# volivan239/raytracing-course-hw

Measured on AMD Instinct MI355X. Metric: Msamples/sec at 1920x1080x256spp, higher is better.
Workload: dtype f32; 1 GPU; synth_room_v1_1920x1080x256; scene=synth_room_v1 (seed 20241223), triangles=268816, emissive_triangles=4204, width=1920, height=1080, spp=256, ray_depth=6, parallelism=pixel tiles 32x32 round-robin over 1 GPU(s), bvh_nodes=265605, bvh_depth=24, light_bvh_depth=19, device_bytes=120573816

## Files before the change

### raytracing-course-hw_amd/csrc/device/rt_persistent.h

```cpp
#pragma once
#include "rt_wavefront.h"

namespace rtamd {
namespace dev {

#define P8_WAVES 4
#define P8_THREADS (64 * P8_WAVES)
#define P8_PER_CU 5
#define PT_MAX_PATHS 5120
#define PT_MIN_GROUP 16
#define PT_NW (PT_MAX_PATHS / 32)
#define PT_BIT_T 1u
#define PT_BIT_L 2u
#define PT_NONE 0xFFFFFFFFu
#define PT_Q_TRACE 0
#define PT_Q_LIGHT 1
#define PT_Q_SHADE 2
#define PT_Q_XLIGHT 3
#define PT_Q_XTRACE 4
#define PT_N_LIVE 5
#define PT_W_TRACE 6
#define PT_W_LIGHT 7
#define PT_GSHIFT 15
#define PT_COST_TRACE_NODE 1u
#define PT_COST_TRACE_TRI 1u
#define PT_COST_LIGHT_NODE 2u
#define PT_COST_LIGHT_TEST 2u
#define PT_COST_SHADE 14u
#define PT_DEBUG_BLOCKS 2048
#define PT_DRAINED 0xFFFFFFFEu
#define PT_T_OVERFLOW (-1.f)
#define PT_WIDE_NONE 0
#define PT_WIDE_WENT 1
#define PT_WIDE_FULL 2
RT_DEV uint32_t pt_near_key(bool entered, uint32_t key) { return entered ? key : 0xFFFFFFFFu; }
RT_DEV void pt_order(uint32_t &ka, uint32_t &ca, uint32_t &kb, uint32_t &cb) {
    const bool s = kb < ka;
    const uint32_t k = s ? kb : ka, c = s ? cb : ca;
    kb = s ? ka : kb; cb = s ? ca : cb;
    ka = k; ca = c;
}
RT_DEV int pt_wide_step_nearest(const GpuNode4Q *nodes, const RayGrid &ray, float cull_t, uint32_t (*stack)[64], int lane, int &sp, int cap, uint32_t &cur) {
    const uint4 *q = reinterpret_cast<const uint4 *>(nodes + cur);
    const uint4 b0 = q[0], b1 = q[1], b2 = q[2], b3 = q[3];
    uint32_t k0, k1, k2, k3;
    const bool h0 = slab_enter_q(b0, ray, cull_t, k0), h1 = slab_enter_q(b1, ray, cull_t, k1);
    const bool h2 = slab_enter_q(b2, ray, cull_t, k2), h3 = slab_enter_q(b3, ray, cull_t, k3);
    k0 = pt_near_key(h0, k0); k1 = pt_near_key(h1, k1); k2 = pt_near_key(h2, k2); k3 = pt_near_key(h3, k3);
    uint32_t c0 = b0.w, c1 = b1.w, c2 = b2.w, c3 = b3.w;
    pt_order(k0, c0, k1, c1); pt_order(k2, c2, k3, c3); pt_order(k0, c0, k2, c2); pt_order(k1, c1, k3, c3); pt_order(k1, c1, k2, c2);
    const int nh = (int)h0 + (int)h1 + (int)h2 + (int)h3;
    if (nh == 0) return PT_WIDE_NONE;
    if (sp + nh - 1 > cap) return PT_WIDE_FULL;
    if (nh > 3) stack[sp++][lane] = c3;
    if (nh > 2) stack[sp++][lane] = c2;
    if (nh > 1) stack[sp++][lane] = c1;
    cur = c0;
    return PT_WIDE_WENT;
}
RT_DEV void pt_wide_enter_all(const GpuNode4Q *nodes, uint32_t cur, const RayGrid &ray, uint4 &b0, uint4 &b1, uint4 &b2, uint4 &b3,
                              bool &h0, bool &h1, bool &h2, bool &h3) {
    const uint4 *q = reinterpret_cast<const uint4 *>(nodes + cur);
    b0 = q[0]; b1 = q[1]; b2 = q[2]; b3 = q[3];
    h0 = slab_test_q(b0, ray); h1 = slab_test_q(b1, ray); h2 = slab_test_q(b2, ray); h3 = slab_test_q(b3, ray);
}
RT_DEV int pt_wide_step_all(const GpuNode4Q *nodes, const RayGrid &ray, uint32_t (*stack)[64], int lane, int &sp, int cap, uint32_t &cur) {
    uint4 b0, b1, b2, b3;
// ... 16 lines not shown
    bool h[4];
    pt_wide_enter_all(S.light_walk_nodes4, 0u, ray, b[0], b[1], b[2], b[3], h[0], h[1], h[2], h[3]);
    steps = 1;
    if (!(h[0] | h[1] | h[2] | h[3])) return 0;
    if (LEVELS < 2) return 2;
    for (int c = 0; c < 4; c++) {
        if (!h[c]) continue;
        if (b[c].w & RT_LEAF_BIT) return 2;
        uint4 g0, g1, g2, g3;
        bool e0, e1, e2, e3;
        pt_wide_enter_all(S.light_walk_nodes4, b[c].w, ray, g0, g1, g2, g3, e0, e1, e2, e3);
        steps++;
        if (e0 | e1 | e2 | e3) return 2;
    }
    return 1;
}
#define PT_EXACT_BATCH 16

struct PtShared {
    uint32_t stack[P8_WAVES][P8_STACK][64];
    uint32_t need[5][PT_NW];
    uint32_t pending[PT_NW * 2];
    uint32_t groups[PT_MAX_PATHS / PT_MIN_GROUP];
    uint32_t cost[PT_MAX_PATHS / PT_MIN_GROUP];
    int cnt[16];
};
static_assert(PT_EXACT_BATCH * RT_STACK_SIZE <= P8_STACK * 64, "the exact role's stacks must fit the wave's LDS stack area");
static_assert(sizeof(PtShared) <= (128 / P8_PER_CU) * 1280, "P8_PER_CU workgroups per CU: the CU's 128 LDS granules of 1,280 bytes shared evenly");

struct PtParams {
    uint32_t n_groups;
    uint32_t group_shift;
    const uint32_t *group_ofs, *group_ids;
    uint32_t *group_cost;
    uint32_t resume;
    int refill, leaf_batch;
    int shade_min;
    int shade_thr0, shade_thr_step;
    int cost_t, cost_l;
    uint32_t front_first;
    int prio;
    unsigned long long deadline_ticks;
    unsigned long long *counters;
    unsigned long long *debug;
    float4 *trace_buf; uint32_t trace_cap; int32_t trace_pixel;
};

struct PtProf {
    unsigned long long t_role[5] = {0, 0, 0, 0, 0};
    unsigned long long iters[2] = {0, 0}, lane_iters[2] = {0, 0}, stints = 0, shade_batches = 0, shade_items = 0;
    unsigned long long t_part[2][3] = {{0, 0, 0}, {0, 0, 0}}, leaf_iters[2] = {0, 0}, leaf_lane_iters[2] = {0, 0}, light_hits = 0, light_tests = 0;
    unsigned long long t_sub[2][3] = {{0, 0, 0}, {0, 0, 0}}, refills[2] = {0, 0};
    unsigned long long light_reach[2] = {0, 0};
};
template <bool COUNT> struct PtLap {
    unsigned long long t;
    RT_DEV PtLap() : t(COUNT ? __builtin_amdgcn_s_memtime() : 0ull) {}
    RT_DEV void lap(unsigned long long &acc) { if (COUNT) { const unsigned long long n = __builtin_amdgcn_s_memtime(); acc += n - t; t = n; } }
};

struct PtWave {
    uint32_t nw, n_local, n_blocks, block;
    bool front_first;
    uint32_t cur[5];
};

template <class SH> RT_DEV uint32_t pt_gshift(const SH &sh) { return (uint32_t)__builtin_amdgcn_readfirstlane(__hip_atomic_load(&sh.cnt[PT_GSHIFT], __ATOMIC_RELAXED, __HIP_MEMORY_SCOPE_WORKGROUP)); }
template <class SH> RT_DEV uint32_t pt_slot(const SH &sh, uint32_t l) { const uint32_t g = pt_gshift(sh); return (sh.groups[l >> g] << g) | (l & ((1u << g) - 1u)); }
RT_DEV int pt_count(const int *p) { return __builtin_amdgcn_readfirstlane(__hip_atomic_load(p, __ATOMIC_RELAXED, __HIP_MEMORY_SCOPE_WORKGROUP)); }

RT_DEV int pt_leaf_batch(int leaf_batch, unsigned long long m_active) {
    const int cap = leaf_batch & 255, share = ((int)__popcll(m_active) * (leaf_batch >> 16) + 255) >> 8;
    return share < cap ? share : cap;
}

RT_DEV unsigned long long pt_ballot(bool p) { return __builtin_amdgcn_ballot_w64(p); }
RT_DEV uint32_t pt_rank_below(unsigned long long m) {
    return __builtin_amdgcn_mbcnt_hi((uint32_t)(m >> 32), __builtin_amdgcn_mbcnt_lo((uint32_t)m, 0u));
}

RT_DEV int pt_prefix(int x, int &total) {
    int before = 0;
    total = 0;
    for (int b = 0; b < 6; b++) {
        if (!pt_ballot((x >> b) != 0)) break;
        const unsigned long long m = pt_ballot((x >> b) & 1);
        before += (int)pt_rank_below(m) << b;
        total += __popcll(m) << b;
    }
    return before;
}

RT_DEV uint32_t pt_pop(uint32_t *bm, int *cnt, const uint32_t nw, uint32_t &cursor, bool want, bool from_start = false) {
    const uint32_t lane = threadIdx.x & 63u;
    if (from_start) cursor = 0u;
    const unsigned long long wantmask = pt_ballot(want);
    const int need = __popcll(wantmask);
    const int my_rank = (int)pt_rank_below(wantmask);
    uint32_t got = PT_NONE;
    int have = 0;
    for (uint32_t swept = 0; swept < nw && have < need; swept += 64u) {
        uint32_t w = cursor + lane;
        const bool valid = lane < nw;
        if (w >= nw) w -= nw;
        const uint32_t v = valid ? bm[w] : 0u;
        const int pc = __popc(v);
        int in_sight;
        const int before = pt_prefix(pc, in_sight);
        uint32_t next_cursor = cursor + 64u;
        if (in_sight) {
            const int room = need - have - before;
            uint32_t take = 0u;
            if (pc > 0 && room > 0) {
                take = v;
                if (room < pc) {
                    uint32_t rest = v;
                    for (int n = room; n > 0; n--) rest &= rest - 1u;
                    take = v & ~rest;
                }
            }
            uint32_t old = 0u;
            if (take) old = atomicAnd(&bm[w], ~take) & take;
            int claimed;
            const int first = pt_prefix(__popc(old), claimed);
            for (unsigned long long cm = pt_ballot(old != 0u); cm; cm &= cm - 1ull) {
                const int j = __ffsll((long long)cm) - 1;
                const uint32_t oj = (uint32_t)__builtin_amdgcn_readlane((int)old, j), wj = (uint32_t)__builtin_amdgcn_readlane((int)w, j);
                const int fj = have + __builtin_amdgcn_readlane(first, j);
                if (want && my_rank >= fj && my_rank < fj + __popc(oj)) {
                    uint32_t bits = oj;
                    for (int k = my_rank - fj; k > 0; k--) bits &= bits - 1u;
                    got = wj * 32u + (uint32_t)__ffs((int)bits) - 1u;
                }
            }
            have += claimed;
            const unsigned long long tm = pt_ballot(take != 0u);
            if (tm && have >= need) {
                const int jl = 63 - __clzll((long long)tm);
                const uint32_t wl = (uint32_t)__builtin_amdgcn_readlane((int)w, jl), left = (uint32_t)__builtin_amdgcn_readlane((int)(v & ~take), jl);
                next_cursor = left ? wl : wl + 1u;
            }
        }
        cursor = (uint32_t)__builtin_amdgcn_readfirstlane((int)next_cursor);
        while (cursor >= nw) cursor -= nw;
    }
    if (have && lane == 0) atomicSub(cnt, have);
    return got;
}

template <class SH> RT_DEV void pt_push(SH &sh, int q, uint32_t l, bool doit) {
    if (doit) atomicOr(&sh.need[q][l >> 5], 1u << (l & 31u));
    const unsigned long long m = pt_ballot(doit);
    if (m && (threadIdx.x & 63u) == 0) atomicAdd(&sh.cnt[q], (int)__popcll(m));
}

template <class SH> RT_DEV void pt_complete(SH &sh, uint32_t l, uint32_t bit, bool doit) {
    bool ready = false;
    if (doit) {
        const uint32_t shift = (l & 15u) * 2u;
        const uint32_t old = atomicAnd(&sh.pending[l >> 4], ~(bit << shift));
        ready = ((old >> shift) & 3u) == bit;
    }
    pt_push(sh, PT_Q_SHADE, l, ready);
}

struct PtTraceQueue {
    static constexpr int ID = PT_Q_TRACE;
    static RT_DEV int refill_at(const PtParams &P) { return P.refill & 0xFFFF; }
    template <class SH> static RT_DEV void publish(SH &sh, uint32_t fin) { pt_complete(sh, fin, PT_BIT_T, fin != PT_NONE); }
};
template <int RARE> struct PtLightQueue {
    static constexpr int ID = PT_Q_LIGHT;
    static RT_DEV int refill_at(const PtParams &P) { return P.refill >> 16; }
    template <class SH> static RT_DEV void publish(SH &sh, uint32_t fin) {
        const bool slow = (fin >> 31) != 0u && fin != PT_NONE;
        pt_complete(sh, fin, PT_BIT_L, fin != PT_NONE && !slow);
        pt_push(sh, RARE, fin & 0x7FFFFFFFu, slow);
    }
};
template <class SH> RT_DEV void pt_book_cost(SH &sh, const PtParams &P, uint32_t l, uint32_t steps) {
    if (P.group_cost) atomicAdd(&sh.cost[l >> pt_gshift(sh)], steps);
}

template <int SLOTS, bool DEFER, bool COUNT, class WK, class SH>
RT_DEV void pt_walk_stint(WK &w, SH &sh, const PtParams &P, PtWave &wv, uint32_t (*stack)[64], const int shade_thr,
                          uint32_t &n_queries, unsigned long long &n_nodes, unsigned long long &n_tris, PtProf &prof) {
    static_assert(SLOTS == 2 || SLOTS == 3, "a lane parks two or three leaves");
    typedef typename WK::Queue Q;
    constexpr int K = Q::ID;
    const int lane = threadIdx.x & 63;
    bool active = false, refill_ok = true, ending = false;
    uint32_t l = 0, slot = 0, cur = 0, fin = PT_NONE;
    int sp = 0;
    uint32_t pend = RT_EMPTY_LEAF, pend2 = RT_EMPTY_LEAF, pend3 = RT_EMPTY_LEAF;
    uint32_t steps = 0;
    auto end_walk = [&]() {
        active = false;
        if (DEFER) ending = true; else fin = w.end(l, slot, steps);
    };
    PtLap<COUNT> clk;
    for (;;) {
        if (DEFER && pt_ballot(ending)) {
            if (ending) { fin = w.end(l, slot, steps); ending = false; }
        }
        const unsigned long long idle = pt_ballot(!active);
        if (idle && (__popcll(idle) >= Q::refill_at(P) || idle == ~0ull)) {
            PtLap<COUNT> sub;
            if (COUNT) prof.refills[K]++;
            if (pt_ballot(fin != PT_NONE)) {
                __builtin_amdgcn_fence(__ATOMIC_RELEASE, "workgroup");
                Q::publish(sh, fin);
                fin = PT_NONE;
            }
            sub.lap(prof.t_sub[K][0]);
            if (!refill_ok) {}
            else if (pt_count(&sh.cnt[PT_Q_SHADE]) >= shade_thr) refill_ok = false;
            else if (pt_count(&sh.cnt[Q::ID]) > 0) {
                const uint32_t got = pt_pop(sh.need[Q::ID], &sh.cnt[Q::ID], wv.nw, wv.cur[Q::ID], !active, wv.front_first);
                __builtin_amdgcn_fence(__ATOMIC_ACQUIRE, "workgroup");
                sub.lap(prof.t_sub[K][1]);
                n_queries += __popcll(pt_ballot(got != PT_NONE));
                if (got != PT_NONE) {
                    l = got; slot = pt_slot(sh, l);
                    w.begin(slot);
                    steps = 0;
                    cur = 0; sp = 0; pend = RT_EMPTY_LEAF; pend2 = RT_EMPTY_LEAF; pend3 = RT_EMPTY_LEAF;
                    active = true;
                }
                sub.lap(prof.t_sub[K][2]);
            }
        }
        const unsigned long long m_active = pt_ballot(active);
        clk.lap(prof.t_part[K][0]);
        if (!m_active) break;
        const int lb = pt_leaf_batch(P.leaf_batch, m_active);
        for (;;) {
            if (active && (cur & RT_LEAF_BIT) && (SLOTS == 3 ? pend3 : pend2) == RT_EMPTY_LEAF && cur != PT_DRAINED) {
                if (pend == RT_EMPTY_LEAF) pend = cur; else if (SLOTS == 2 || pend2 == RT_EMPTY_LEAF) pend2 = cur; else pend3 = cur;
                cur = sp == 0 ? PT_DRAINED : stack[--sp][lane];
                if (cur == PT_DRAINED && pend == RT_EMPTY_LEAF) end_walk();
            }
            const bool inner = active && !(cur & RT_LEAF_BIT);
            if (!pt_ballot(inner) || __popcll(pt_ballot(active && (cur & RT_LEAF_BIT))) >= lb) break;
            if (COUNT) { prof.iters[K]++; prof.lane_iters[K] += __popcll(pt_ballot(inner)); }
            if (inner) {
                if (COUNT) n_nodes++;
                steps += WK::COST_NODE;
                const int went = w.step(cur, sp);
                if (went == PT_WIDE_NONE) {
                    if (sp != 0) cur = stack[--sp][lane];
                    else if (pend != RT_EMPTY_LEAF) cur = PT_DRAINED;
                    else end_walk();
                } else if (went == PT_WIDE_FULL) {
                    w.full();
                    pend = RT_EMPTY_LEAF; pend2 = RT_EMPTY_LEAF; pend3 = RT_EMPTY_LEAF;
                    end_walk();
                }
            }
        }
        clk.lap(prof.t_part[K][1]);
        const bool at_leaf = active && pend != RT_EMPTY_LEAF;
        if (COUNT) { prof.leaf_iters[K]++; prof.leaf_lane_iters[K] += __popcll(pt_ballot(at_leaf)); }
        if (at_leaf) {
            uint32_t i = pend & ~RT_LEAF_BIT, more = pend2, more2 = pend3;
            typename WK::Leaf lf;
            for (;;) {
                const bool last = w.test(i, sp, lf);
                if (COUNT) n_tris++;
                steps += WK::COST_TEST;
                if (!last) i++;
                else if (more == RT_EMPTY_LEAF) break;
// ... 367 lines not shown
template <class RL>
RT_DEV void pt_run(RL &rl) {
    constexpr bool COUNT = RL::COUNT;
    auto &sh = rl.sh;
    const RenderView &R = rl.R;
    const PtParams &P = rl.P;
    const uint32_t tid = threadIdx.x, lane = tid & 63u;
    const uint32_t wave = (uint32_t)__builtin_amdgcn_readfirstlane((int)(tid >> 6));
    PtWave wv;
    if (!pt_enter<RL::THREADS>(sh, P, wv)) return;

    for (uint32_t base = 0; base < wv.n_local; base += RL::THREADS) {
        const uint32_t l = base + tid;
        bool started = false, wire = false;
        if (l < wv.n_local) {
            const uint32_t slot = pt_slot(sh, l), gslot = slot + rl.W.slot_base;
            int x, y; Rng rng; F3 sum;
            if (wf_seed_record(R, gslot, !P.resume, x, y, rng, sum)) {
                if (P.resume) started = rl.resumed_sample(slot) < (uint32_t)R.samples;
                else { rl.seed(slot, gslot, x, y, rng, sum); started = true; }
                if (started) {
                    atomicOr(&sh.pending[l >> 4], PT_BIT_T << ((l & 15u) * 2u));
                    wire = rl.seed_wire(slot);
                }
            }
        }
        const unsigned long long m = pt_ballot(started);
        if (m && lane == 0) atomicAdd(&sh.cnt[PT_N_LIVE], (int)__popcll(m));
        pt_push(sh, PT_Q_TRACE, l, started && !wire);
        pt_push(sh, PT_Q_XTRACE, l, wire);
    }
    __builtin_amdgcn_fence(__ATOMIC_RELEASE, "workgroup");
    __syncthreads();
    __builtin_amdgcn_fence(__ATOMIC_ACQUIRE, "workgroup");

    uint32_t(*stack)[64] = rl.stack;
    const int shade_thr = P.shade_thr0 + (int)wave * P.shade_thr_step;
    uint32_t n_closest = 0, n_light = 0;
    unsigned long long n_nodes = 0, n_tris = 0;
    uint32_t idle_spins = 0;
    int gave_up = 0;
    PtProf prof;
    PtLap<COUNT> clk;
    const unsigned long long t_start = __builtin_amdgcn_s_memrealtime();
    for (;;) {
        if (__builtin_amdgcn_s_memrealtime() - t_start > P.deadline_ticks) { gave_up = 1; break; }
        const int ns = pt_count(&sh.cnt[PT_Q_SHADE]), nt = pt_count(&sh.cnt[PT_Q_TRACE]), nl = pt_count(&sh.cnt[PT_Q_LIGHT]);
        if (rl.rare(wv)) {
            idle_spins = 0;
            clk.lap(prof.t_role[3]);
            continue;
        }
        if (ns >= P.shade_min || (ns > 0 && nt + nl == 0)) {
            const uint32_t got = pt_pop(sh.need[PT_Q_SHADE], &sh.cnt[PT_Q_SHADE], wv.nw, wv.cur[PT_Q_SHADE], true, wv.front_first);
            __builtin_amdgcn_fence(__ATOMIC_ACQUIRE, "workgroup");
            if (pt_here(P.prio) == 2) __builtin_amdgcn_s_setprio(2);
            const PtShaded s = rl.shade(got, n_light, n_nodes, prof);
            __builtin_amdgcn_fence(__ATOMIC_RELEASE, "workgroup");
            if (s.trace || s.light) atomicOr(&sh.pending[got >> 4], ((s.trace ? PT_BIT_T : 0u) | (s.light ? PT_BIT_L : 0u)) << ((got & 15u) * 2u));
            pt_push(sh, PT_Q_TRACE, got, s.trace && !s.xtrace);
            pt_push(sh, PT_Q_LIGHT, got, s.light);
            pt_push(sh, PT_Q_XTRACE, got, s.xtrace);
            if (s.cost) atomicAdd(&sh.cost[got >> pt_gshift(sh)], s.cost);
            const unsigned long long done = pt_ballot(s.done);
            if (done && lane == 0) atomicSub(&sh.cnt[PT_N_LIVE], (int)__popcll(done));
            idle_spins = 0;
            if (pt_here(P.prio) == 2) __builtin_amdgcn_s_setprio(0);
            if (COUNT) { prof.shade_batches++; prof.shade_items += __popcll(pt_ballot(got != PT_NONE)); }
            clk.lap(prof.t_role[2]);
            continue;
        }
        if (nt + nl > 0) {
            const long long wt = (long long)nt * P.cost_t * (pt_count(&sh.cnt[PT_W_LIGHT]) + 1), wl = (long long)nl * P.cost_l * (pt_count(&sh.cnt[PT_W_TRACE]) + 1);
            if (pt_here(P.prio) == 1) __builtin_amdgcn_s_setprio(2);
            if (nl == 0 || (nt > 0 && wt >= wl)) {
                if (lane == 0) atomicAdd(&sh.cnt[PT_W_TRACE], 1);
                auto walk = rl.trace_walk();
                pt_walk_stint<RL::SLOTS, RL::DEFER, COUNT>(walk, sh, P, wv, stack, shade_thr, n_closest, n_nodes, n_tris, prof);
                if (lane == 0) atomicSub(&sh.cnt[PT_W_TRACE], 1);
                clk.lap(prof.t_role[0]);
            } else {
                if (lane == 0) atomicAdd(&sh.cnt[PT_W_LIGHT], 1);
                auto walk = rl.light_walk(prof);
                pt_walk_stint<RL::SLOTS, RL::DEFER, COUNT>(walk, sh, P, wv, stack, shade_thr, n_light, n_nodes, n_tris, prof);
                if (lane == 0) atomicSub(&sh.cnt[PT_W_LIGHT], 1);
                clk.lap(prof.t_role[1]);
            }
            if (pt_here(P.prio) == 1) __builtin_amdgcn_s_setprio(0);
            idle_spins = 0;
            if (COUNT) prof.stints++;
            continue;
        }
        if (pt_count(&sh.cnt[PT_N_LIVE]) <= 0) break;
        __builtin_amdgcn_s_sleep(8);
        clk.lap(prof.t_role[4]);
        if (++idle_spins > (1u << 24)) { gave_up = 2; break; }
    }
    if (gave_up && lane == 0 && P.counters) atomicAdd(&P.counters[gave_up == 1 ? CNT_DEADLINE : CNT_LOST_PATH], 1ull);
    pt_leave<RL::THREADS>(sh, P, wv);
    if (P.counters) {
        if (lane == 0 && n_closest) atomicAdd(&P.counters[CNT_CLOSEST], (unsigned long long)n_closest);
        if (lane == 0 && n_light) atomicAdd(&P.counters[CNT_LIGHT], (unsigned long long)n_light);
        if (COUNT) {
            atomicAdd(&P.counters[CNT_NODE_VISITS], n_nodes); atomicAdd(&P.counters[CNT_TRI_TESTS], n_tris);
            if (lane == 0) for (int i = 0; i < 5; i++) atomicAdd(&P.counters[CNT_ROLE_TIME + i], prof.t_role[i]);
        }
        rl.flush(lane, prof);
// ... 45 lines not shown
            if (tin && ty * R.width + tx == P.trace_pixel) {
                const float4 *tr = wf_rec(W, tslot);
                const uint32_t k = atomicAdd(reinterpret_cast<uint32_t *>(P.trace_buf), 1u);
                if (4u * k + 5u <= P.trace_cap) for (int q = 0; q < 4; q++) P.trace_buf[1 + 4 * k + q] = tr[q];
            }
        }
        if (got != PT_NONE) { PtPark pk; pk.p = (PtLdsWord)&stack[0][lane]; todo = pt_shade_lean<FEAT>(S, R, W, pt_slot(sh, got), pk, discarded); }
        n_discarded += __popcll(pt_ballot(discarded));
        const bool next = got != PT_NONE && todo != PT_SHADE_EXACT && (todo & WF_NEXT_TRACE), with_light = next && (todo & WF_NEXT_LIGHT);
        bool wire = false;
        bool settled = false;
        int settle_steps = 0;
        if (next && (S.n_tripwire_groups || ((COUNT || PT_LIGHT_SETTLE) && with_light))) {
            const float4 *nr = wf_rec(W, pt_slot(sh, got));
            const float4 n0 = nr[0], n1 = nr[1];
            const F3 o = f3(n0.x, n0.y, n0.z), d = f3(n0.w, n1.x, n1.y);
            if (S.n_tripwire_groups) wire = pt_tripwire(S, o, d);
            if ((COUNT || PT_LIGHT_SETTLE) && with_light) {
                const int reach = pt_light_reach<COUNT ? 2 : PT_LIGHT_SETTLE>(S, make_ray_grid(S.grid, o, d), settle_steps);
                if (COUNT) { prof.light_reach[0] += reach == 0; prof.light_reach[1] += reach == 1; }
                settled = reach < PT_LIGHT_SETTLE;
                if (settled) {
                    const int depth = (int)(__float_as_uint(reinterpret_cast<const float *>(nr + 3)[3]) & 15u);
                    float *pdf = reinterpret_cast<float *>(wf_entry(W, pt_slot(sh, got), depth)) + 3;
                    *pdf = *pdf + 0.f / S.n_lights_f;
                }
            }
        }
        n_light += __popcll(pt_ballot(settled));
        if (COUNT && settled) n_nodes += (unsigned long long)settle_steps;
        PtShaded s;
        s.trace = next;
        s.light = with_light && !settled;
        s.xtrace = (got != PT_NONE && todo == PT_SHADE_EXACT) || wire;
        s.done = got != PT_NONE && (todo == 0 || todo == WF_PARKED);
        if (got != PT_NONE && todo != PT_SHADE_EXACT) s.cost = (uint32_t)PT_COST_SHADE + (settled ? PT_COST_LIGHT_NODE * (uint32_t)settle_steps : 0u);
        return s;
    }
    RT_DEV void flush(uint32_t lane, const PtProf &prof) {
        if (lane == 0) {
            if (n_discarded) atomicAdd(&P.counters[CNT_DISCARDED], (unsigned long long)n_discarded);
            if (n_xtrace) atomicAdd(&P.counters[CNT_EXACT_CLOSEST], (unsigned long long)n_xtrace);
            if (n_xlight) atomicAdd(&P.counters[CNT_EXACT_LIGHT], (unsigned long long)n_xlight);
        }
        if (!COUNT) return;
        atomicAdd(&P.counters[CNT_P8_LIGHT_HITS], prof.light_hits); atomicAdd(&P.counters[CNT_P8_LIGHT_TESTS], prof.light_tests);
        atomicAdd(&P.counters[CNT_P8_LIGHT_REACH], prof.light_reach[0]); atomicAdd(&P.counters[CNT_P8_LIGHT_REACH + 1], prof.light_reach[1]);
        if (lane == 0) {
            atomicAdd(&P.counters[CNT_P8_WALK_ITERS], prof.iters[0]); atomicAdd(&P.counters[CNT_P8_WALK_ITERS + 1], prof.lane_iters[0]);
            atomicAdd(&P.counters[CNT_P8_WALK_ITERS + 2], prof.iters[1]); atomicAdd(&P.counters[CNT_P8_WALK_ITERS + 3], prof.lane_iters[1]);
            atomicAdd(&P.counters[CNT_P8_STINTS], prof.stints); atomicAdd(&P.counters[CNT_P8_SHADE_BATCHES], prof.shade_batches); atomicAdd(&P.counters[CNT_P8_SHADE_ITEMS], prof.shade_items);
            for (int k = 0; k < 3; k++) atomicAdd(&P.counters[CNT_P8_HANDOFF_TIME + k], prof.t_sub[0][k]);
            atomicAdd(&P.counters[CNT_P8_HANDOFFS], prof.refills[0]);
            for (int w = 0; w < 2; w++) {
                for (int k = 0; k < 3; k++) atomicAdd(&P.counters[CNT_P8_WALK_TIME + 3 * w + k], prof.t_part[w][k]);
                atomicAdd(&P.counters[CNT_P8_LEAF_ITERS + 2 * w], prof.leaf_iters[w]); atomicAdd(&P.counters[CNT_P8_LEAF_ITERS + 2 * w + 1], prof.leaf_lane_iters[w]);
            }
        }
    }
};

template <bool COUNT, int FEAT>
__global__ __launch_bounds__(P8_THREADS, P8_PER_CU) void pt_persistent_kernel(SceneView S, RenderView R, WfView W, PtParams P) {
    __shared__ PtShared sh;
    PtRoles<COUNT, FEAT> roles{S, R, W, sh, P};
    pt_run(roles);
}

}
}
```

### raytracing-course-hw_amd/csrc/device/rt_types.h

```cpp
#pragma once
#include <stdint.h>

namespace rtamd {

#define RT_MAX_DEPTH 16
#define RT_STACK_SIZE 64
#define P8_STACK 24

enum CounterSlot {
    CNT_CLOSEST = 0,
    CNT_LIGHT = 1,
    CNT_NODE_VISITS = 2,
    CNT_TRI_TESTS = 3,
    CNT_WF_NODE_ITERS = 4,
    CNT_WF_LEAF_PHASES = 5,
    CNT_WF_LEAF_LANES = 6,
    CNT_WF_REFILLS = 7,
    CNT_WF_LANE_NODES = 8,
    CNT_WF_LANE_TRIS = 9,
    CNT_DISCARDED = 10,
    CNT_WF_SLOW_LIGHT = 11,
    CNT_P6_EXACT_LIGHT = 11,
    CNT_EXACT_CLOSEST = 12,
    CNT_EXACT_LIGHT = 13,
    CNT_P6_SLOW_LIGHT = 13,
    CNT_LOST_PATH = 14,
    CNT_WANT_HISTOGRAMS = 15,
    CNT_WF_HIST_CLOSEST = 16,
    CNT_ROLE_TIME = 16,
    CNT_P8_WALK_ITERS = 21,
    CNT_P8_STINTS = 25,
    CNT_P8_SHADE_BATCHES = 26,
    CNT_P8_SHADE_ITEMS = 27,
    CNT_DEADLINE = 29,
    CNT_P8_LIGHT_REACH = 30,
    CNT_WF_HIST_LIGHT = 32,
    CNT_P6_SLOW_HITS = 32,
    CNT_P8_WALK_TIME = 48,
    CNT_P8_LEAF_ITERS = 54,
    CNT_P8_LIGHT_HITS = 58,
    CNT_P8_LIGHT_TESTS = 59,
    CNT_P8_HANDOFF_TIME = 60,
    CNT_P8_HANDOFFS = 63,
    CNT_SLOTS = 64
};
#define CNT_BYTES (CNT_SLOTS * sizeof(unsigned long long))

struct GpuNode {
    float lo0[3]; int32_t child0;
    float hi0[3]; int32_t cnt0;
    float lo1[3]; int32_t child1;
    float hi1[3]; int32_t cnt1;
};
static_assert(sizeof(GpuNode) == 64, "GpuNode must be 64 bytes");

struct GpuNode4Q { uint32_t rec[4][4]; };
static_assert(sizeof(GpuNode4Q) == 64, "GpuNode4Q must be 64 bytes");
#define RT_GRID_CELLS 65000.0
#define RT_GRID_BORDER 4
struct NodeGrid { float lo[3], step[3], istep[3]; };

struct TriIsect {
    float ax, ay, az;
    float nx, ny, nz;
    float a1, b1;
    float a2, b2;
    float den;
    uint32_t pad;
};
static_assert(sizeof(TriIsect) == 48, "TriIsect must be 48 bytes");

struct TriShade {
    float n3[3], dn1[3], dn2[3];
    float t3[3], dt1[3], dt2[3];
    float uv3[2], duv1[2], duv2[2];
    float tanw;
    uint32_t material;
    uint32_t orig;
    uint32_t pad;
};
static_assert(sizeof(TriShade) == 112, "TriShade must be 112 bytes");

struct LightRec {
    TriIsect isect;
    float b[3], c[3];
    float point_prob;
    float n3[3], dn1[3], dn2[3];
    float box_lo[3], pad0;
    float box_hi[3], pad1;
};
// ... 81 lines not shown
```

### raytracing-course-hw_amd/csrc/rtamd_api.hip

```cpp
#include <hip/hip_runtime.h>
#include <algorithm>
#include <cmath>
#include <cstdio>
#include <cstring>
#include <functional>
#include <memory>
#include <string>
#include <vector>
#include "../../include/rtamd.h"
#include "host/knobs.h"
#include "host/rt_scene.h"
#include "host/rt_accum_state.h"
#include "device/rt_kernels_hw8.h"
#include "device/rt_wavefront.h"
#include "device/rt_persistent.h"
#include "device/rt_kernels_hw6.h"
#include "device/rt_persistent_hw6.h"
#include "device/rt_kernels_txt.h"
#include "device/rt_kernels_hw2.h"
#include "device/rt_kernels_hw4.h"
#include "device/rt_kernels_hw5.h"

using namespace rtamd;

// ... 377 lines not shown
    const char *ksel = env_str("RTAMD_KERNEL");
    const bool mega = ksel && strcmp(ksel, "mega") == 0;
    rounds_chosen = ksel && strcmp(ksel, "wavefront") == 0;
    switch (integrator) {
    case RT_INTEGRATOR_HW1: return Pipeline::Hw1;
    case RT_INTEGRATOR_HW2: return Pipeline::Hw2;
    case RT_INTEGRATOR_HW3: return Pipeline::Hw3;
    case RT_INTEGRATOR_HW4: return Pipeline::Hw4;
    case RT_INTEGRATOR_HW5: return Pipeline::Hw5;
    }
    if (scene->flavor == RT_INTEGRATOR_HW6)
        return scene->hw6_pt_stack && !mega && !env_flag("RTAMD_HW6_SCRATCH_STACK") ? Pipeline::Persistent6 : Pipeline::Mega6;
    const rt_scene_info &I = scene->info;
    if (mega || I.bvh_depth > WF_STACK + WF_OVF || I.light_bvh_depth > 64 || I.n_triangles >= 0x40000000u
        || R.samples / streams >= (1 << 25))
        return Pipeline::Mega8;
    if (rounds_chosen || I.bvh_depth > P8_STACK || scene->light_walk_depth > P8_STACK || env_flag("RTAMD_WF_LDS_STACK")) return Pipeline::Rounds;
    const uint64_t auto_groups = (uint64_t)env_int("RTAMD_AUTO_GROUPS_PER_CU", 0);
    if (!ksel && auto_groups && (uint64_t)n_work * (uint64_t)streams >= auto_groups * (uint64_t)scene->n_cus) return Pipeline::Rounds;
    return Pipeline::Persistent8;
}

static void report_persistent(rt_scene *scene, bool hw6, const char *kernel, bool count, const unsigned long long *h_cnt) {
    const bool times = scene->d_pt_debug && scene->pt_blocks <= PT_DEBUG_BLOCKS;
    const unsigned long long *role = h_cnt + CNT_ROLE_TIME;
    const double tt = (double)(role[0] + role[1] + role[2] + role[3] + role[4]);
    auto nz = [](unsigned long long d) { return (double)(d ? d : 1); };
    if (hw6) {
        fprintf(stderr, "[rtamd] persistent hw6 pipeline: %u launches; re-deal %.2f ms on the host (slowest workgroup / mean under the round-robin deal: %.3f); light sums through the slow role %llu of %llu; exact closest-hit walks %llu of %llu, exact light sums %llu\n",
                scene->pt_launches, scene->pt_rebalance_ms, scene->pt_imbalance, h_cnt[CNT_P6_SLOW_LIGHT], h_cnt[CNT_LIGHT], h_cnt[CNT_EXACT_CLOSEST], h_cnt[CNT_CLOSEST], h_cnt[CNT_P6_EXACT_LIGHT]);
        if (count) {
            fprintf(stderr, "[rtamd] persistent hw6 kernel, light sums in the slow role by number of hits (0..14, 15+):");
            for (int b = 0; b < 16; b++) fprintf(stderr, " %llu", h_cnt[CNT_P6_SLOW_HITS + b]);
            fprintf(stderr, "\n");
            fprintf(stderr, "[rtamd] persistent hw6 kernel, wave time by role: closest-hit walks %.1f %%, light walks %.1f %%, shading %.1f %%, slow light sums %.1f %%, idle %.1f %%\n",
                    100 * role[0] / tt, 100 * role[1] / tt, 100 * role[2] / tt, 100 * role[3] / tt, 100 * role[4] / tt);
        }
    } else if (times && count) {
        const unsigned long long *iters = h_cnt + CNT_P8_WALK_ITERS, n_light = h_cnt[CNT_LIGHT];
        fprintf(stderr, "[rtamd] persistent kernel, wave time by role: closest-hit walks %.1f %%, light walks %.1f %%, shading %.1f %%, exact walks %.2f %%, idle %.1f %%; "
                        "walker lane utilisation: closest hit %.1f of 64 (%llu wave iterations), light %.1f of 64 (%llu); %llu stints, %llu shade batches of %.1f paths\n",
                100 * role[0] / tt, 100 * role[1] / tt, 100 * role[2] / tt, 100 * role[3] / tt, 100 * role[4] / tt,
                (double)iters[1] / nz(iters[0]), iters[0], (double)iters[3] / nz(iters[2]), iters[2],
                h_cnt[CNT_P8_STINTS], h_cnt[CNT_P8_SHADE_BATCHES], (double)h_cnt[CNT_P8_SHADE_ITEMS] / nz(h_cnt[CNT_P8_SHADE_BATCHES]));
        for (int w = 0; w < 2; w++) {
            const unsigned long long *part = h_cnt + CNT_P8_WALK_TIME + 3 * w, *leaf = h_cnt + CNT_P8_LEAF_ITERS + 2 * w;
            const double tw = (double)(part[0] + part[1] + part[2]);
            fprintf(stderr, "[rtamd]   %s walker's wave time: hand-off and refill %.1f %%, inner nodes %.1f %%, leaves %.1f %%; leaf passes %llu with %.1f of 64 lanes\n",
                    w ? "light" : "closest-hit", 100 * part[0] / tw, 100 * part[1] / tw, 100 * part[2] / tw, leaf[0], (double)leaf[1] / nz(leaf[0]));
        }
        const unsigned long long *handoff = h_cnt + CNT_P8_HANDOFF_TIME, tests = h_cnt[CNT_P8_LIGHT_TESTS], hits = h_cnt[CNT_P8_LIGHT_HITS], *reach = h_cnt + CNT_P8_LIGHT_REACH;
        fprintf(stderr, "[rtamd]   closest-hit walker's hand-off points: %llu; of their time: publishing finished walks %.1f %%, taking new ones from the bitmap %.1f %%, reading their rays %.1f %% (the rest: the test itself)\n",
                h_cnt[CNT_P8_HANDOFFS], 100.0 * handoff[0] / nz(h_cnt[CNT_P8_WALK_TIME]), 100.0 * handoff[1] / nz(h_cnt[CNT_P8_WALK_TIME]), 100.0 * handoff[2] / nz(h_cnt[CNT_P8_WALK_TIME]));
        fprintf(stderr, "[rtamd]   light tests %llu (%.2f per light sum), hits %llu (%.2f per light sum); triangle tests of closest-hit walks %llu (%.2f per query)\n",
                tests, (double)tests / nz(n_light), hits, (double)hits / nz(n_light), h_cnt[CNT_TRI_TESTS] - tests, (double)(h_cnt[CNT_TRI_TESTS] - tests) / nz(h_cnt[CNT_CLOSEST]));
        fprintf(stderr, "[rtamd]   light sums whose walk ends at the light tree's root %llu (%.1f %%), one level below it %llu (%.1f %%); settled by the shader: level %d\n",
                reach[0], 100.0 * reach[0] / nz(n_light), reach[1], 100.0 * reach[1] / nz(n_light), PT_LIGHT_SETTLE);
    }
    if (!times) return;
    std::vector<unsigned long long> dbg((size_t)scene->pt_blocks * 3);
    HIP_CHECK(hipMemcpy(dbg.data(), scene->d_pt_debug, dbg.size() * sizeof(unsigned long long), hipMemcpyDeviceToHost));
    unsigned long long t0 = ~0ull, tmin = ~0ull, tmax = 0; double tsum = 0;
    for (uint32_t b = 0; b < scene->pt_blocks; b++) if (dbg[3 * b] && dbg[3 * b] < t0) t0 = dbg[3 * b];
    for (uint32_t b = 0; b < scene->pt_blocks; b++) { unsigned long long e = dbg[3 * b + 1] - t0; tmin = e < tmin ? e : tmin; tmax = e > tmax ? e : tmax; tsum += (double)e; }
    if (const char *dump = env_str("RTAMD_DUMP_WG")) {
        if (FILE *f = fopen(dump, "w")) {
            for (uint32_t b = 0; b < scene->pt_blocks; b++) fprintf(f, "%u %.4f %.4f %llu\n", b, (dbg[3 * b] - t0) * 1e-5, (dbg[3 * b + 1] - t0) * 1e-5, dbg[3 * b + 2]);
            fclose(f);
        }
    }
    if (!hw6)
        fprintf(stderr, "[rtamd] persistent pipeline: %u launches; re-deal of the sub-tiles took %.2f ms on the host (slowest workgroup / mean under the round-robin deal: %.3f)\n",
                scene->pt_launches, scene->pt_rebalance_ms, scene->pt_imbalance);
    fprintf(stderr, "[rtamd] %s (last launch): %u workgroups, exit times min / mean / max = %.3f / %.3f / %.3f ms after the first start",
            kernel, scene->pt_blocks, tmin * 1e-5, tsum / scene->pt_blocks * 1e-5, tmax * 1e-5);
    if (!hw6) fprintf(stderr, "; exact closest hits %llu, exact light sums %llu of %llu + %llu queries", h_cnt[CNT_EXACT_CLOSEST], h_cnt[CNT_EXACT_LIGHT], h_cnt[CNT_CLOSEST], h_cnt[CNT_LIGHT]);
    fprintf(stderr, "\n");
}

static const char *accum_unsupported(Pipeline pipe, const rt_render_params *p) {
    if (p->sample_streams > 1) return "throughput mode (sample_streams > 1) has no resumable state";
    if (p->flags & ~RT_FLAG_COUNTERS) return "flags other than RT_FLAG_COUNTERS do not apply to a resumable render (the outputs are named at rt_accum_resolve)";
    switch (pipe) {
    case Pipeline::Persistent8: case Pipeline::Persistent6: case Pipeline::Rounds: return nullptr;
    case Pipeline::Mega8: return "the hw8 / hw7 megakernel is in effect (RTAMD_KERNEL=mega, or a tree beyond the persistent and round kernels' limits): a resumable render needs the persistent or the round pipeline";
    case Pipeline::Mega6: return "the hw6 per-lane path machine is in effect (RTAMD_KERNEL=mega, RTAMD_HW6_SCRATCH_STACK, or a tree beyond the persistent hw6 kernel's stacks): a resumable render needs the persistent hw6 pipeline";
    default: return "the hw1 .. hw5 integrators have no resumable state (RT_INTEGRATOR_HW6 / HW7 / HW8 only)";
    }
}

struct AccumSlice { uint32_t *state; int32_t first; };

struct Frame {
    RenderView R{};
    SceneView V8{};
    Pipeline pipe = Pipeline::Persistent8;
    bool rounds_chosen = false, count = false, time_trace = false;
    uint32_t n_work = 0;
    uint32_t blocks = 0;
    int streams = 1;
    float txt_tan_fov_y = 0;
    uint32_t launches = 0;
};

static const int max_ray_depth[RT_INTEGRATOR_HW8 + 1] = {0, RT_MAX_DEPTH, RT2_MAX_DEPTH, RT3_MAX_DEPTH, RT4_MAX_DEPTH, RT4_MAX_DEPTH, RT6_MAX_DEPTH, RT_MAX_DEPTH, RT_MAX_DEPTH};

// ... 419 lines not shown
```

Baseline: 480.9 Msamples/s.

## Speed up bitmap queue pop with DPP prefix scans and lane permutes

Moves the persistent kernel's bitmap queue pop into its own header and rewrites its wave-level pieces. The bit-serial ballot prefix sum becomes a DPP inclusive scan, the nth-set-bit selection uses a binary popcount search instead of a loop, and the per-lane serial rank matching is replaced by ds_permute/bpermute scatter-gather. The second prefix scan is skipped when every atomic claim succeeded. It also adds optional pop statistics counters, which only run in counting mode. The risk is subtle correctness issues in the DPP row masks and the permute routing.

```diff
diff --git a/raytracing-course-hw_amd/csrc/device/rt_persistent.h b/raytracing-course-hw_amd/csrc/device/rt_persistent.h
--- a/raytracing-course-hw_amd/csrc/device/rt_persistent.h
+++ b/raytracing-course-hw_amd/csrc/device/rt_persistent.h
@@ -1,5 +1,6 @@
 #pragma once
 #include "rt_wavefront.h"
+#include "rt_pt_queue.h"
 
 namespace rtamd {
 namespace dev {
@@ -12,7 +13,6 @@
 #define PT_NW (PT_MAX_PATHS / 32)
 #define PT_BIT_T 1u
 #define PT_BIT_L 2u
-#define PT_NONE 0xFFFFFFFFu
 #define PT_Q_TRACE 0
 #define PT_Q_LIGHT 1
 #define PT_Q_SHADE 2
@@ -135,6 +135,7 @@
     unsigned long long t_part[2][3] = {{0, 0, 0}, {0, 0, 0}}, leaf_iters[2] = {0, 0}, leaf_lane_iters[2] = {0, 0}, light_hits = 0, light_tests = 0;
     unsigned long long t_sub[2][3] = {{0, 0, 0}, {0, 0, 0}}, refills[2] = {0, 0};
     unsigned long long light_reach[2] = {0, 0};
+    PtPopStat pops[3];
 };
 template <bool COUNT> struct PtLap {
     unsigned long long t;
@@ -150,91 +151,9 @@
 
 template <class SH> RT_DEV uint32_t pt_gshift(const SH &sh) { return (uint32_t)__builtin_amdgcn_readfirstlane(__hip_atomic_load(&sh.cnt[PT_GSHIFT], __ATOMIC_RELAXED, __HIP_MEMORY_SCOPE_WORKGROUP)); }
 template <class SH> RT_DEV uint32_t pt_slot(const SH &sh, uint32_t l) { const uint32_t g = pt_gshift(sh); return (sh.groups[l >> g] << g) | (l & ((1u << g) - 1u)); }
-RT_DEV int pt_count(const int *p) { return __builtin_amdgcn_readfirstlane(__hip_atomic_load(p, __ATOMIC_RELAXED, __HIP_MEMORY_SCOPE_WORKGROUP)); }
-
 RT_DEV int pt_leaf_batch(int leaf_batch, unsigned long long m_active) {
     const int cap = leaf_batch & 255, share = ((int)__popcll(m_active) * (leaf_batch >> 16) + 255) >> 8;
     return share < cap ? share : cap;
-}
-
-RT_DEV unsigned long long pt_ballot(bool p) { return __builtin_amdgcn_ballot_w64(p); }
-RT_DEV uint32_t pt_rank_below(unsigned long long m) {
-    return __builtin_amdgcn_mbcnt_hi((uint32_t)(m >> 32), __builtin_amdgcn_mbcnt_lo((uint32_t)m, 0u));
-}
-
-RT_DEV int pt_prefix(int x, int &total) {
-    int before = 0;
-    total = 0;
-    for (int b = 0; b < 6; b++) {
-        if (!pt_ballot((x >> b) != 0)) break;
-        const unsigned long long m = pt_ballot((x >> b) & 1);
-        before += (int)pt_rank_below(m) << b;
-        total += __popcll(m) << b;
-    }
-    return before;
-}
-
-RT_DEV uint32_t pt_pop(uint32_t *bm, int *cnt, const uint32_t nw, uint32_t &cursor, bool want, bool from_start = false) {
-    const uint32_t lane = threadIdx.x & 63u;
-    if (from_start) cursor = 0u;
-    const unsigned long long wantmask = pt_ballot(want);
-    const int need = __popcll(wantmask);
-    const int my_rank = (int)pt_rank_below(wantmask);
-    uint32_t got = PT_NONE;
-    int have = 0;
-    for (uint32_t swept = 0; swept < nw && have < need; swept += 64u) {
-        uint32_t w = cursor + lane;
-        const bool valid = lane < nw;
-        if (w >= nw) w -= nw;
-        const uint32_t v = valid ? bm[w] : 0u;
-        const int pc = __popc(v);
-        int in_sight;
-        const int before = pt_prefix(pc, in_sight);
-        uint32_t next_cursor = cursor + 64u;
-        if (in_sight) {
-            const int room = need - have - before;
-            uint32_t take = 0u;
-            if (pc > 0 && room > 0) {
-                take = v;
-                if (room < pc) {
-                    uint32_t rest = v;
-                    for (int n = room; n > 0; n--) rest &= rest - 1u;
-                    take = v & ~rest;
-                }
-            }
-            uint32_t old = 0u;
-            if (take) old = atomicAnd(&bm[w], ~take) & take;
-            int claimed;
-            const int first = pt_prefix(__popc(old), claimed);
-            for (unsigned long long cm = pt_ballot(old != 0u); cm; cm &= cm - 1ull) {
-                const int j = __ffsll((long long)cm) - 1;
-                const uint32_t oj = (uint32_t)__builtin_amdgcn_readlane((int)old, j), wj = (uint32_t)__builtin_amdgcn_readlane((int)w, j);
-                const int fj = have + __builtin_amdgcn_readlane(first, j);
-                if (want && my_rank >= fj && my_rank < fj + __popc(oj)) {
-                    uint32_t bits = oj;
-                    for (int k = my_rank - fj; k > 0; k--) bits &= bits - 1u;
-                    got = wj * 32u + (uint32_t)__ffs((int)bits) - 1u;
-                }
-            }
-            have += claimed;
-            const unsigned long long tm = pt_ballot(take != 0u);
-            if (tm && have >= need) {
-                const int jl = 63 - __clzll((long long)tm);
-                const uint32_t wl = (uint32_t)__builtin_amdgcn_readlane((int)w, jl), left = (uint32_t)__builtin_amdgcn_readlane((int)(v & ~take), jl);
-                next_cursor = left ? wl : wl + 1u;
-            }
-        }
-        cursor = (uint32_t)__builtin_amdgcn_readfirstlane((int)next_cursor);
-        while (cursor >= nw) cursor -= nw;
-    }
-    if (have && lane == 0) atomicSub(cnt, have);
-    return got;
-}
-
-template <class SH> RT_DEV void pt_push(SH &sh, int q, uint32_t l, bool doit) {
-    if (doit) atomicOr(&sh.need[q][l >> 5], 1u << (l & 31u));
-    const unsigned long long m = pt_ballot(doit);
-    if (m && (threadIdx.x & 63u) == 0) atomicAdd(&sh.cnt[q], (int)__popcll(m));
 }
 
 template <class SH> RT_DEV void pt_complete(SH &sh, uint32_t l, uint32_t bit, bool doit) {
@@ -299,7 +218,7 @@
             if (!refill_ok) {}
             else if (pt_count(&sh.cnt[PT_Q_SHADE]) >= shade_thr) refill_ok = false;
             else if (pt_count(&sh.cnt[Q::ID]) > 0) {
-                const uint32_t got = pt_pop(sh.need[Q::ID], &sh.cnt[Q::ID], wv.nw, wv.cur[Q::ID], !active, wv.front_first);
+                const uint32_t got = pt_pop(sh.need[Q::ID], &sh.cnt[Q::ID], wv.nw, wv.cur[Q::ID], !active, wv.front_first, COUNT ? &prof.pops[K] : nullptr);
                 __builtin_amdgcn_fence(__ATOMIC_ACQUIRE, "workgroup");
                 sub.lap(prof.t_sub[K][1]);
                 n_queries += __popcll(pt_ballot(got != PT_NONE));
@@ -773,7 +692,7 @@
             continue;
         }
         if (ns >= P.shade_min || (ns > 0 && nt + nl == 0)) {
-            const uint32_t got = pt_pop(sh.need[PT_Q_SHADE], &sh.cnt[PT_Q_SHADE], wv.nw, wv.cur[PT_Q_SHADE], true, wv.front_first);
+            const uint32_t got = pt_pop(sh.need[PT_Q_SHADE], &sh.cnt[PT_Q_SHADE], wv.nw, wv.cur[PT_Q_SHADE], true, wv.front_first, COUNT ? &prof.pops[PT_Q_SHADE] : nullptr);
             __builtin_amdgcn_fence(__ATOMIC_ACQUIRE, "workgroup");
             if (pt_here(P.prio) == 2) __builtin_amdgcn_s_setprio(2);
             const PtShaded s = rl.shade(got, n_light, n_nodes, prof);
@@ -925,6 +844,10 @@
             atomicAdd(&P.counters[CNT_P8_STINTS], prof.stints); atomicAdd(&P.counters[CNT_P8_SHADE_BATCHES], prof.shade_batches); atomicAdd(&P.counters[CNT_P8_SHADE_ITEMS], prof.shade_items);
             for (int k = 0; k < 3; k++) atomicAdd(&P.counters[CNT_P8_HANDOFF_TIME + k], prof.t_sub[0][k]);
             atomicAdd(&P.counters[CNT_P8_HANDOFFS], prof.refills[0]);
+            for (int q = 0; q < 3; q++) {
+                atomicAdd(&P.counters[CNT_P8_POPS + 3 * q], prof.pops[q].pops); atomicAdd(&P.counters[CNT_P8_POPS + 3 * q + 1], prof.pops[q].paths);
+                atomicAdd(&P.counters[CNT_P8_POPS + 3 * q + 2], prof.pops[q].words);
+            }
             for (int w = 0; w < 2; w++) {
                 for (int k = 0; k < 3; k++) atomicAdd(&P.counters[CNT_P8_WALK_TIME + 3 * w + k], prof.t_part[w][k]);
                 atomicAdd(&P.counters[CNT_P8_LEAF_ITERS + 2 * w], prof.leaf_iters[w]); atomicAdd(&P.counters[CNT_P8_LEAF_ITERS + 2 * w + 1], prof.leaf_lane_iters[w]);
diff --git a/raytracing-course-hw_amd/csrc/device/rt_pt_queue.h b/raytracing-course-hw_amd/csrc/device/rt_pt_queue.h
--- /dev/null
+++ b/raytracing-course-hw_amd/csrc/device/rt_pt_queue.h
@@ -0,0 +1,107 @@
+#pragma once
+#include <hip/hip_runtime.h>
+#include <stdint.h>
+
+#ifndef RT_DEV
+#define RT_DEV __device__ __forceinline__
+#endif
+#define PT_NONE 0xFFFFFFFFu
+
+namespace rtamd {
+namespace dev {
+
+__host__ __device__ inline int pt_nth_bit(uint32_t v, int n) {
+    int pos = 0;
+#pragma unroll
+    for (int h = 16; h > 0; h >>= 1) {
+        const int c = __builtin_popcount((v >> pos) & ((1u << h) - 1u));
+        if (n >= c) { n -= c; pos += h; }
+    }
+    return pos;
+}
+__host__ __device__ inline uint32_t pt_low_bits(uint32_t v, int n) { return v & ((2u << pt_nth_bit(v, n - 1)) - 1u); }
+
+RT_DEV int pt_count(const int *p) { return __builtin_amdgcn_readfirstlane(__hip_atomic_load(p, __ATOMIC_RELAXED, __HIP_MEMORY_SCOPE_WORKGROUP)); }
+
+RT_DEV unsigned long long pt_ballot(bool p) { return __builtin_amdgcn_ballot_w64(p); }
+RT_DEV uint32_t pt_rank_below(unsigned long long m) {
+    return __builtin_amdgcn_mbcnt_hi((uint32_t)(m >> 32), __builtin_amdgcn_mbcnt_lo((uint32_t)m, 0u));
+}
+
+template <int CTRL, int ROW_MASK> RT_DEV int pt_dpp_or_zero(int x) { return __builtin_amdgcn_update_dpp(0, x, CTRL, ROW_MASK, 0xf, false); }
+RT_DEV int pt_prefix(int x, int &total) {
+    int s = x;
+    s += pt_dpp_or_zero<0x111, 0xf>(s);
+    s += pt_dpp_or_zero<0x112, 0xf>(s);
+    s += pt_dpp_or_zero<0x114, 0xf>(s);
+    s += pt_dpp_or_zero<0x118, 0xf>(s);
+    s += pt_dpp_or_zero<0x142, 0xa>(s);
+    s += pt_dpp_or_zero<0x143, 0xc>(s);
+    total = __builtin_amdgcn_readlane(s, 63);
+    return s - x;
+}
+
+struct PtPopStat {
+    unsigned long long pops = 0, paths = 0, words = 0;
+};
+
+RT_DEV uint32_t pt_pop(uint32_t *bm, int *cnt, const uint32_t nw, uint32_t &cursor, bool want, bool from_start = false, PtPopStat *stat = nullptr) {
+    const uint32_t lane = threadIdx.x & 63u;
+    if (from_start) cursor = 0u;
+    const unsigned long long wantmask = pt_ballot(want);
+    const int need = __popcll(wantmask);
+    uint32_t box = 0u;
+    int have = 0;
+    for (uint32_t swept = 0; swept < nw && have < need; swept += 64u) {
+        uint32_t w = cursor + lane;
+        const bool valid = lane < nw;
+        if (w >= nw) w -= nw;
+        const uint32_t v = valid ? bm[w] : 0u;
+        const int pc = __popc(v);
+        int in_sight;
+        const int before = pt_prefix(pc, in_sight);
+        uint32_t next_cursor = cursor + 64u;
+        if (in_sight) {
+            const int open = need - have, room = open - before;
+            uint32_t take = 0u;
+            if (pc > 0 && room > 0) take = room < pc ? pt_low_bits(v, room) : v;
+            uint32_t old = 0u;
+            if (take) old = atomicAnd(&bm[w], ~take) & take;
+            int claimed = in_sight < open ? in_sight : open, first = before < open ? before : open;
+            if (pt_ballot(old != take)) first = pt_prefix(__popc(old), claimed);
+            const unsigned long long cm = pt_ballot(old != 0u);
+            for (unsigned long long m = cm; m; m &= m - 1ull) {
+                const int j = __ffsll((long long)m) - 1;
+                const uint32_t oj = (uint32_t)__builtin_amdgcn_readlane((int)old, j), wj = (uint32_t)__builtin_amdgcn_readlane((int)w, j);
+                const uint32_t fj = (uint32_t)(have + __builtin_amdgcn_readlane(first, j));
+                const bool mine = __builtin_amdgcn_inverse_ballot_w64((unsigned long long)oj);
+                const uint32_t rank = __builtin_amdgcn_mbcnt_lo(oj, fj), behind = (fj + (uint32_t)__popc(oj)) & 63u;
+                const uint32_t to = mine ? rank : behind;
+                box |= (uint32_t)__builtin_amdgcn_ds_permute((int)(to << 2), mine ? (int)(wj * 32u + lane + 1u) : 0);
+            }
+            have += claimed;
+            if (stat) stat->words += __popcll(cm);
+            const unsigned long long tm = pt_ballot(take != 0u);
+            if (tm && have >= need) {
+                const int jl = 63 - __clzll((long long)tm);
+                const uint32_t wl = (uint32_t)__builtin_amdgcn_readlane((int)w, jl), left = (uint32_t)__builtin_amdgcn_readlane((int)(v & ~take), jl);
+                next_cursor = left ? wl : wl + 1u;
+            }
+        }
+        cursor = (uint32_t)__builtin_amdgcn_readfirstlane((int)next_cursor);
+        while (cursor >= nw) cursor -= nw;
+    }
+    if (have && lane == 0) atomicSub(cnt, have);
+    if (stat) { stat->pops++; stat->paths += (unsigned long long)have; }
+    const uint32_t got = (uint32_t)__builtin_amdgcn_ds_bpermute((int)(pt_rank_below(wantmask) << 2), (int)box) - 1u;
+    return want ? got : PT_NONE;
+}
+
+template <class SH> RT_DEV void pt_push(SH &sh, int q, uint32_t l, bool doit) {
+    if (doit) atomicOr(&sh.need[q][l >> 5], 1u << (l & 31u));
+    const unsigned long long m = pt_ballot(doit);
+    if (m && (threadIdx.x & 63u) == 0) atomicAdd(&sh.cnt[q], (int)__popcll(m));
+}
+
+}
+}
diff --git a/raytracing-course-hw_amd/csrc/device/rt_types.h b/raytracing-course-hw_amd/csrc/device/rt_types.h
--- a/raytracing-course-hw_amd/csrc/device/rt_types.h
+++ b/raytracing-course-hw_amd/csrc/device/rt_types.h
@@ -36,6 +36,7 @@
     CNT_P8_LIGHT_REACH = 30,
     CNT_WF_HIST_LIGHT = 32,
     CNT_P6_SLOW_HITS = 32,
+    CNT_P8_POPS = 32,
     CNT_P8_WALK_TIME = 48,
     CNT_P8_LEAF_ITERS = 54,
     CNT_P8_LIGHT_HITS = 58,
diff --git a/raytracing-course-hw_amd/csrc/rtamd_api.hip b/raytracing-course-hw_amd/csrc/rtamd_api.hip
--- a/raytracing-course-hw_amd/csrc/rtamd_api.hip
+++ b/raytracing-course-hw_amd/csrc/rtamd_api.hip
@@ -453,6 +453,11 @@
         const unsigned long long *handoff = h_cnt + CNT_P8_HANDOFF_TIME, tests = h_cnt[CNT_P8_LIGHT_TESTS], hits = h_cnt[CNT_P8_LIGHT_HITS], *reach = h_cnt + CNT_P8_LIGHT_REACH;
         fprintf(stderr, "[rtamd]   closest-hit walker's hand-off points: %llu; of their time: publishing finished walks %.1f %%, taking new ones from the bitmap %.1f %%, reading their rays %.1f %% (the rest: the test itself)\n",
                 h_cnt[CNT_P8_HANDOFFS], 100.0 * handoff[0] / nz(h_cnt[CNT_P8_WALK_TIME]), 100.0 * handoff[1] / nz(h_cnt[CNT_P8_WALK_TIME]), 100.0 * handoff[2] / nz(h_cnt[CNT_P8_WALK_TIME]));
+        for (int q = 0; q < 3; q++) {
+            const unsigned long long *pop = h_cnt + CNT_P8_POPS + 3 * q;
+            fprintf(stderr, "[rtamd]   pops of the %s queue: %llu, %.1f paths from %.2f claimed words each\n", q == 0 ? "closest-hit" : q == 1 ? "light" : "shade",
+                    pop[0], (double)pop[1] / nz(pop[0]), (double)pop[2] / nz(pop[0]));
+        }
         fprintf(stderr, "[rtamd]   light tests %llu (%.2f per light sum), hits %llu (%.2f per light sum); triangle tests of closest-hit walks %llu (%.2f per query)\n",
                 tests, (double)tests / nz(n_light), hits, (double)hits / nz(n_light), h_cnt[CNT_TRI_TESTS] - tests, (double)(h_cnt[CNT_TRI_TESTS] - tests) / nz(h_cnt[CNT_CLOSEST]));
         fprintf(stderr, "[rtamd]   light sums whose walk ends at the light tree's root %llu (%.1f %%), one level below it %llu (%.1f %%); settled by the shader: level %d\n",
```

Measured after the change: 503.9 Msamples/s (median of 6 runs). 1.05x the previous value.
